# marksho-sfdc/TransmogrifAI

Hardware: AMD Instinct MI355X
Metric: end-to-end AutoML wall-clock + hold-out AuPR, 10M-row binary-class tabular (lower is better)
Workload: dtype fp32; 1 GPU; binary-10m; model=BinaryClassificationModelSelector(default grid), rows=10000000, raw_columns=200, cv_folds=3, global_batch=10000000, max_training_sample=1000000, parallelism=single

## Files before the change

### transmogrifai_amd/ops/csrc/hip/tree_kernels.hip

```cpp
#include <hip/hip_runtime.h>
#include <algorithm>
#include <cstdlib>
#include <stdint.h>
#include <math.h>

#define TM_MAX_S 16
#define TM_WIDE_MAX_S 256
#define TM_WIDE_MAX_BS 16384

namespace {

struct HistItem {
  int32_t node;
  int32_t fg0;
  int32_t nf;
  int32_t excl;
  int64_t begin;
  int64_t count;
};

__device__ __forceinline__ uint32_t ent_row(uint32_t e, int wide) { return wide ? e : (e & 0xFFFFFFu); }
__device__ __forceinline__ uint32_t ent_w(uint32_t e, int wide) { return wide ? 1u : (e >> 24); }

template <int MODE>
// ... 513 lines not shown
      const int f = k / (B * S);
      if (k - f * (B * S) >= wlimit) continue;
      const int64_t acc = lds[f * rowstride + (k - f * (B * S))];
      if (excl) out[k] = acc;
      else if (acc != 0) atomicAdd(reinterpret_cast<unsigned long long*>(out + k), (unsigned long long)acc);
    }
    return;
  }
  const int cwords = FG * B * sc;
  for (int k = threadIdx.x; k < cwords; k += blockDim.x) {
    const int f = k / (B * sc);
    const int rem = k - f * (B * sc);
    int64_t acc = 0;
    for (int r = 0; r < R; ++r) acc += lds[(r * FG + f) * rowstride + rem];
    const int bin = rem / sc, c = rem - bin * sc;
    int64_t* w = out + ((int64_t)f * B + bin) * S + s0 + c;
    if (excl) *w = acc;
    else if (acc != 0) atomicAdd(reinterpret_cast<unsigned long long*>(w), (unsigned long long)acc);
  }
  }
}

__device__ __forceinline__ int64_t live_words(int64_t sz, int64_t dense, int per, int S) {
  return (dense < 0 || sz <= dense) ? sz : dense + (sz - dense) / per * S;
}
__device__ __forceinline__ int live_word(int k, int dense, int per, int S) {
  if (dense < 0 || k < dense) return k;
  const int t = k - dense, f = t / S;
  return dense + f * per + (t - f * S);
}

__global__ void hist_subtract_kernel(int64_t* __restrict__ hist, const int64_t* __restrict__ parent,
                                     const int64_t* __restrict__ parent_off, const int64_t* __restrict__ small_off,
                                     const int64_t* __restrict__ out_off, const int64_t* __restrict__ size, int n,
                                     int64_t dense, int per, int S) {
  const int j = blockIdx.y;
  if (j >= n) return;
  const int sz = (int)live_words(size[j], dense, per, S);
  const int dn = (int)dense;
  const int64_t* p = parent + parent_off[j];
  const int64_t* s = hist + small_off[j];
  int64_t* o = hist + out_off[j];
  for (int k = blockIdx.x * blockDim.x + threadIdx.x; k < sz; k += gridDim.x * blockDim.x) {
    const int w = live_word(k, dn, per, S);
    o[w] = p[w] - s[w];
  }
}

__global__ void zero_segments_kernel(int64_t* __restrict__ hist, const int64_t* __restrict__ off,
                                     const int64_t* __restrict__ size, int n, int64_t dense, int per, int S,
                                     int n_dense, const int* __restrict__ dcnt) {
  const int j = blockIdx.y;
  if (dcnt != nullptr) {
    n = dcnt[0];
    n_dense = dcnt[1];
  }
  if (j >= n) return;
  int64_t* o = hist + off[j];
  const int64_t dj = j < n_dense ? dense : 0;
  const int sz = (int)live_words(size[j], dj, per, S);
  const int dn = (int)dj;
  for (int k = blockIdx.x * blockDim.x + threadIdx.x; k < sz; k += gridDim.x * blockDim.x)
    o[live_word(k, dn, per, S)] = 0;
}

#pragma clang fp contract(off)
__device__ __forceinline__ double impurity_dev(const double* st, int S, int kind, double* cnt) {
  if (kind == 0 || kind == 1) {
    double n = 0;
    for (int s = 0; s < S; ++s) n += st[s];
    *cnt = n;
    if (n <= 0) return 0.0;
    double imp = kind == 0 ? 1.0 : 0.0;
    for (int s = 0; s < S; ++s) {
      const double p = st[s] / n;
      if (kind == 0) imp -= p * p;
      else if (p > 0) imp -= p * log2(p);
    }
    return imp;
  }
  if (kind == 2) {
    const double n = st[0];
    *cnt = n;
    if (n <= 0) return 0.0;
    const double m = st[1] / n;
    return st[2] / n - m * m;
  }
  *cnt = st[1];
  return 0.0;
}

#define TM_FOR_S(s) _Pragma("unroll") for (int s = 0; s < SM; ++s) if (s < S)

template <int SM>
__device__ __forceinline__ double impurity_reg(const double* st, int S, int kind, double* cnt) {
  if (kind == 0 || kind == 1) {
    double n = 0;
    TM_FOR_S(s) n += st[s];
    *cnt = n;
    if (n <= 0) return 0.0;
    double imp = kind == 0 ? 1.0 : 0.0;
    TM_FOR_S(s) {
      const double p = st[s] / n;
      if (kind == 0) imp -= p * p;
      else if (p > 0) imp -= p * log2(p);
    }
    return imp;
  }
  if (kind == 2) {
    const double n = st[0];
    *cnt = n;
    if (n <= 0) return 0.0;
    const double m = st[1] / n;
    return st[2] / n - m * m;
  }
  *cnt = st[1];
  return 0.0;
}

struct Best {
  double gain;
  int f;
  int b;
  int dl;
};
static_assert(sizeof(Best) == 24, "candidate record: three 8-byte words (store_best_sc1 / load_best_sc1)");

__device__ __forceinline__ void store_best_sc1(Best* p, const Best& b) {
  uint64_t* w = reinterpret_cast<uint64_t*>(p);
  __hip_atomic_store(w, (uint64_t)__double_as_longlong(b.gain), __ATOMIC_RELAXED, __HIP_MEMORY_SCOPE_AGENT);
  __hip_atomic_store(w + 1, (uint64_t)(uint32_t)b.f | ((uint64_t)(uint32_t)b.b << 32), __ATOMIC_RELAXED,
                     __HIP_MEMORY_SCOPE_AGENT);
  __hip_atomic_store(w + 2, (uint64_t)(uint32_t)b.dl, __ATOMIC_RELAXED, __HIP_MEMORY_SCOPE_AGENT);
}
__device__ __forceinline__ Best load_best_sc1(const Best* p) {
  const uint64_t* w = reinterpret_cast<const uint64_t*>(p);
  const uint64_t g = __hip_atomic_load(w, __ATOMIC_RELAXED, __HIP_MEMORY_SCOPE_AGENT);
  const uint64_t fb = __hip_atomic_load(w + 1, __ATOMIC_RELAXED, __HIP_MEMORY_SCOPE_AGENT);
  const uint64_t dl = __hip_atomic_load(w + 2, __ATOMIC_RELAXED, __HIP_MEMORY_SCOPE_AGENT);
  return Best{__longlong_as_double((long long)g), (int)(uint32_t)fb, (int)(uint32_t)(fb >> 32), (int)(uint32_t)dl};
}

__device__ __forceinline__ bool better(const Best& a, const Best& b) {
  if (a.gain != b.gain) return a.gain > b.gain;
  if (a.f != b.f) return a.f < b.f;
  if (a.dl != b.dl) return a.dl < b.dl;
  return a.b < b.b;
}

constexpr int FPB = 16;

static inline int cand_stride(int fbmax) { return (fbmax + 15) & ~15; }

static int split_fpb() {
  static const int v = [] {
    const char* e = std::getenv("TMOG_SPLIT_FPB");
    const int x = e ? std::atoi(e) : FPB;
    return (x == 4 || x == 8 || x == 16) ? x : FPB;
  }();
  return v;
}

struct ReduceArgs {
  const int64_t* hist;
  const int64_t* node_hist_off;
  const int32_t* node_feat_off;
  const int32_t* feat_list;
  int B, S, missing_bin;
  const int32_t* node_model;
  const double* qinv;
  int fbmax;
  int cstride;
  const Best* cand;
  int32_t* out_feat;
  int32_t* out_bin;
  float* out_gain;
  uint8_t* out_dl;
  float* out_left;
  float* out_total;
  unsigned long long* cursors;
  uint8_t* rec;
  int64_t rec_bytes;
  int fp_mlo, fp_nml, fp_obase;
};

__device__ __forceinline__ void reduce_node(const ReduceArgs& ra, int j, int lane, bool sc1 = false) {
  const int B = ra.B, S = ra.S, fbmax = ra.fbmax, missing_bin = ra.missing_bin;
  if (ra.cursors && lane < 2) ra.cursors[2 * j + lane] = 0;
  Best b{-INFINITY, 0x7fffffff, 0, 0};
  for (int i = lane; i < fbmax; i += 64) {
    const Best* cp = ra.cand + (int64_t)j * ra.cstride + i;
    const Best c = sc1 ? load_best_sc1(cp) : *cp;
    if (better(c, b)) b = c;
  }
  for (int off = 32; off > 0; off >>= 1) {
    Best o;
    o.gain = __shfl_xor(b.gain, off, 64);
    o.f = __shfl_xor(b.f, off, 64);
    o.b = __shfl_xor(b.b, off, 64);
    o.dl = __shfl_xor(b.dl, off, 64);
    if (better(o, b)) b = o;
  }
  const bool found = b.f != 0x7fffffff && b.gain > -INFINITY;
  const int64_t* h = ra.hist + ra.node_hist_off[j];
  const double* qi = ra.qinv + (int64_t)(ra.node_model ? ra.node_model[j] : 0) * S;
  if (lane == 0) {
    ra.out_feat[j] = found ? ra.feat_list[ra.node_feat_off[j] + b.f] : -1;
    ra.out_bin[j] = found ? b.b : -1;
    ra.out_gain[j] = found ? (float)b.gain : -INFINITY;
    ra.out_dl[j] = (uint8_t)(found ? b.dl : 0);
  }
  for (int s = 0; s < S; ++s) {
    int64_t t = 0, l = 0;
    const int64_t* hf = h + (int64_t)(found ? b.f : 0) * B * S;
    for (int bb = lane; bb < B; bb += 64) {
      t += h[(int64_t)bb * S + s];
      if (found && bb <= b.b) l += hf[(int64_t)bb * S + s];
    }
    if (found && b.dl && lane == 0) l += hf[(int64_t)missing_bin * S + s];
    for (int off = 32; off > 0; off >>= 1) {
      t += __shfl_xor(t, off, 64);
      l += __shfl_xor(l, off, 64);
    }
    if (lane == 0) {
      ra.out_total[(int64_t)j * S + s] = (float)((double)t * qi[s]);
      ra.out_left[(int64_t)j * S + s] = (float)((double)l * qi[s]);
      if (ra.rec) reinterpret_cast<float*>(ra.rec + (int64_t)j * ra.rec_bytes + 24)[s] = (float)((double)l * qi[s]);
    }
  }
  if (ra.rec && lane == 0) {
    uint8_t* r = ra.rec + (int64_t)j * ra.rec_bytes;
    *reinterpret_cast<double*>(r) = found ? b.gain : -INFINITY;
    reinterpret_cast<int32_t*>(r)[2] =
        found ? (b.f < ra.fp_nml ? ra.fp_mlo + b.f : ra.fp_obase + (b.f - ra.fp_nml)) : 0x7fffffff;
    reinterpret_cast<int32_t*>(r)[3] = found ? b.b : -1;
    reinterpret_cast<int32_t*>(r)[4] = found ? b.dl : 0;
    reinterpret_cast<int32_t*>(r)[5] = found ? ra.feat_list[ra.node_feat_off[j] + b.f] : -1;
  }
}

template <int SM>
struct NodeScan {
  int64_t totq[SM];
  double tot[SM], q[SM];
  double tcount, pimp, parent_gain, min_inst, min_gain, mcw, lambda;
  int S, kind;
  bool allow_missing;
  Best best;

  __device__ __forceinline__ void init(const int64_t* totq_in, const double* qi, const float* P, int S_, int kind_,
                                       int missing_bin) {
    S = S_;
    kind = kind_;
    best = Best{-INFINITY, 0x7fffffff, 0, 0};
    min_inst = P[0];
    min_gain = P[1];
    mcw = P[2];
    lambda = P[3];
    allow_missing = P[5] > 0.5f && missing_bin >= 0;
    TM_FOR_S(s) {
      totq[s] = totq_in[s];
      q[s] = qi[s];
      tot[s] = (double)totq[s] * q[s];
    }
    pimp = impurity_reg<SM>(tot, S, kind, &tcount);
    parent_gain = kind == 3 ? tot[0] * tot[0] / (tot[1] + lambda) : 0.0;
  }

  __device__ __forceinline__ void consider(const int64_t* lq, int f, int b, int dl) {
    double left[SM], right[SM];
    TM_FOR_S(s) {
      left[s] = (double)lq[s] * q[s];
      right[s] = (double)(totq[s] - lq[s]) * q[s];
    }
    double gain;
    bool ok = true;
    if (kind == 3) {
      if (left[1] < mcw || right[1] < mcw) return;
      gain = left[0] * left[0] / (left[1] + lambda) + right[0] * right[0] / (right[1] + lambda) - parent_gain;
    } else {
      double lc, rc;
      const double li = impurity_reg<SM>(left, S, kind, &lc);
      const double ri = impurity_reg<SM>(right, S, kind, &rc);
      if (lc < min_inst || rc < min_inst || lc <= 0 || rc <= 0) ok = false;
      gain = pimp - (lc / tcount) * li - (rc / tcount) * ri;
      if (gain < min_gain) ok = false;
    }
    if (ok) {
      Best c{gain, f, b, dl};
      if (better(c, best)) best = c;
    }
  }

  __device__ __forceinline__ void scan_feature(int64_t* v, const int64_t* miss, int nb, int f, int lane) {
    TM_FOR_S(s) v[s] = wave_scan64(v[s]);
    bool any_miss = false;
    TM_FOR_S(s) any_miss |= miss[s] != 0;
    const int n_dl = allow_missing ? (any_miss ? 2 : 1) : 1;
    if (lane < nb - 1 + (allow_missing ? 1 : 0)) {
      for (int dl = 0; dl < n_dl; ++dl) {
        if (lane == nb - 1 && dl) continue;
        int64_t lq[SM];
        TM_FOR_S(s) lq[s] = v[s] + (dl ? miss[s] : 0);
        consider(lq, f, lane, dl);
      }
    }
  }

  __device__ __forceinline__ void wave_best() {
    for (int off = 32; off > 0; off >>= 1) {
      Best o;
      o.gain = __shfl_xor(best.gain, off, 64);
      o.f = __shfl_xor(best.f, off, 64);
      o.b = __shfl_xor(best.b, off, 64);
      o.dl = __shfl_xor(best.dl, off, 64);
      if (better(o, best)) best = o;
    }
  }
};

template <int SM>
__device__ __forceinline__ void node_totals(const int64_t* h, int B, int S, int lane, int64_t* totq) {
  int64_t v[SM];
  TM_FOR_S(s) v[s] = lane < B ? h[lane * S + s] : 0;
  TM_FOR_S(s) totq[s] = readlane64(wave_scan64(v[s]), 63);
}

template <int SM>
__global__ void __launch_bounds__(256) split_scan_kernel(
    const int64_t* __restrict__ hist, const int64_t* __restrict__ node_hist_off, const int32_t* __restrict__ node_nfeat,
    const int32_t* __restrict__ node_feat_off, const int32_t* __restrict__ feat_list,
    const int32_t* __restrict__ feat_nbins, int B, int S, int kind, const float* __restrict__ node_params,
    int missing_bin, const int32_t* __restrict__ node_model, const double* __restrict__ qinv, int fbmax,
    Best* __restrict__ cand, int n_multi, int fpb, unsigned* __restrict__ done, ReduceArgs ra,
    const int* __restrict__ dm) {
  const int cstride = ra.cstride;
  const int j = blockIdx.x / fbmax;
  const int fb = blockIdx.x - j * fbmax;
  if (dm != nullptr && j >= *dm) return;
  const int lane = threadIdx.x & 63, wave = threadIdx.x >> 6;
  if (node_params[(int64_t)j * 8 + 4] > 0.5f) {
    if (done && fb == 0 && wave == 0) reduce_node(ra, j, lane);
    return;
  }
  const int nf = node_nfeat[j];
  const int f_lim = n_multi >= 0 ? min(n_multi, nf) : nf;
  const int fb_multi = n_multi >= 0 ? (n_multi + fpb - 1) / fpb : fbmax;
  const bool one_blk = fb >= fb_multi;
  __shared__ Best s_best[4];
  NodeScan<SM> ns;
  ns.best = Best{-INFINITY, 0x7fffffff, 0, 0};
  if (node_params[(int64_t)j * 8 + 7] > 0.5f &&
      (one_blk ? (n_multi + (fb - fb_multi) * 256 < nf) : (fb * fpb < f_lim))) {
    const int64_t* h = hist + node_hist_off[j];
    const int32_t* fl = feat_list + node_feat_off[j];
    int64_t totq[SM];
    node_totals<SM>(h, B, S, lane, totq);
    ns.init(totq, qinv + (int64_t)(node_model ? node_model[j] : 0) * S, node_params + (int64_t)j * 8, S, kind,
            missing_bin);
    const int f_end = one_blk ? 0 : min(f_lim, (fb + 1) * fpb);
    if (one_blk) {
      const int f = n_multi + (fb - fb_multi) * 256 + (int)threadIdx.x;
      if (f < nf && ns.allow_missing && feat_nbins[fl[f]] == 1) {
        const int64_t* hf = h + (int64_t)f * B * S;
        int64_t lq[SM];
        TM_FOR_S(s) lq[s] = hf[s];
        ns.consider(lq, f, 0, 0);
      }
    }
    for (int f = fb * fpb + wave; f < f_end; f += 4) {
      const int nb = feat_nbins[fl[f]];
      const int64_t* hf = h + (int64_t)f * B * S;
      if (nb == 1) {
        if (ns.allow_missing && lane == 0) {
          int64_t lq[SM];
          TM_FOR_S(s) lq[s] = hf[s];
          ns.consider(lq, f, 0, 0);
        }
        continue;
      }
      int64_t v[SM], miss[SM];
      const int bl = lane < nb ? lane : 0;
      const int mbin = missing_bin >= 0 ? missing_bin : 0;
      TM_FOR_S(s) {
        v[s] = hf[bl * S + s];
        miss[s] = hf[mbin * S + s];
      }
      TM_FOR_S(s) {
        v[s] = lane < nb ? v[s] : 0;
        miss[s] = ns.allow_missing ? miss[s] : 0;
      }
      ns.scan_feature(v, miss, nb, f, lane);
    }
  }
  ns.wave_best();
  if (lane == 0) s_best[wave] = ns.best;
  __syncthreads();
  if (done == nullptr) {
    if (threadIdx.x == 0) {
      Best b = s_best[0];
      for (int w = 1; w < 4; ++w)
        if (better(s_best[w], b)) b = s_best[w];
      cand[(int64_t)j * cstride + fb] = b;
    }
    return;
  }
  if (wave == 0) {
    unsigned last = 0;
    if (lane == 0) {
      Best b = s_best[0];
      for (int w = 1; w < 4; ++w)
        if (better(s_best[w], b)) b = s_best[w];
      store_best_sc1(cand + (int64_t)j * cstride + fb, b);
      asm volatile("s_waitcnt vmcnt(0)" ::: "memory");
      last = __hip_atomic_fetch_add(done + j, 1u, __ATOMIC_RELAXED, __HIP_MEMORY_SCOPE_AGENT) ==
             (unsigned)(fbmax - 1);
    }
    last = __shfl(last, 0, 64);
    if (last) {
      reduce_node(ra, j, lane, true);
      if (lane == 0) __hip_atomic_store(done + j, 0u, __ATOMIC_RELAXED, __HIP_MEMORY_SCOPE_AGENT);
    }
  }
}

template <int SM>
__global__ void __launch_bounds__(256) pair_scan_kernel(
    int64_t* __restrict__ hist, const int64_t* __restrict__ parent, const int64_t* __restrict__ parent_off,
    const int32_t* __restrict__ small_j, const int32_t* __restrict__ big_j, int n_pairs,
    const int64_t* __restrict__ node_hist_off, const int32_t* __restrict__ node_nfeat,
    const int32_t* __restrict__ node_feat_off, const int32_t* __restrict__ feat_list,
    const int32_t* __restrict__ feat_nbins, int B, int S, int kind, const float* __restrict__ node_params,
    int missing_bin, const int32_t* __restrict__ node_model, const double* __restrict__ qinv, int fbmax,
    Best* __restrict__ cand, int n_multi, int fpb, int cstride, const int* __restrict__ dnp) {
  const int q = blockIdx.x / fbmax;
  const int fb = blockIdx.x - q * fbmax;
  if (dnp != nullptr) n_pairs = *dnp;
  if (q >= n_pairs) return;
  const int lane = threadIdx.x & 63, wave = threadIdx.x >> 6;
  const int js = small_j[q], jb = big_j[q];
  const int nf = node_nfeat[js];
  const int f_lim = n_multi >= 0 ? min(n_multi, nf) : nf;
  const int fb_multi = n_multi >= 0 ? (n_multi + fpb - 1) / fpb : fbmax;
  const bool one_blk = fb >= fb_multi;
  const int64_t* P = parent + parent_off[q];
  const int64_t* Hs = hist + node_hist_off[js];
  int64_t* Hb = hist + node_hist_off[jb];
  const int32_t* fl = feat_list + node_feat_off[js];
  const bool scan_s = node_params[(int64_t)js * 8 + 7] > 0.5f;
  const bool scan_b = node_params[(int64_t)jb * 8 + 7] > 0.5f;
  __shared__ Best s_best[2][4];
  NodeScan<SM> ns, nb_;
  {
    int64_t ts[SM], tp[SM], tb[SM];
    node_totals<SM>(Hs, B, S, lane, ts);
    node_totals<SM>(P, B, S, lane, tp);
    TM_FOR_S(s) tb[s] = tp[s] - ts[s];
    ns.init(ts, qinv + (int64_t)(node_model ? node_model[js] : 0) * S, node_params + (int64_t)js * 8, S, kind,
            missing_bin);
    nb_.init(tb, qinv + (int64_t)(node_model ? node_model[jb] : 0) * S, node_params + (int64_t)jb * 8, S, kind,
             missing_bin);
  }
  if (one_blk) {
    const int f = n_multi + (fb - fb_multi) * 256 + (int)threadIdx.x;
    if (f < nf) {
      const int64_t o = (int64_t)f * B * S;
      int64_t ls[SM], lb[SM];
      TM_FOR_S(s) {
        ls[s] = Hs[o + s];
        lb[s] = P[o + s] - ls[s];
        Hb[o + s] = lb[s];
      }
      if (feat_nbins[fl[f]] == 1) {
        if (scan_s && ns.allow_missing) ns.consider(ls, f, 0, 0);
        if (scan_b && nb_.allow_missing) nb_.consider(lb, f, 0, 0);
      }
    }
  } else {
    const int f_end = min(f_lim, (fb + 1) * fpb);
    for (int f = fb * fpb + wave; f < f_end; f += 4) {
      const int nbins = feat_nbins[fl[f]];
      const int64_t o = (int64_t)f * B * S;
      int64_t vs[SM], vb[SM], ms[SM], mb[SM], pa[SM], pp[SM];
      const int bl = lane < B ? lane : 0;
      TM_FOR_S(s) {
        pa[s] = Hs[o + bl * S + s];
        pp[s] = P[o + bl * S + s];
      }
      TM_FOR_S(s) {
        const int64_t a = lane < B ? pa[s] : 0;
        const int64_t c = lane < B ? pp[s] - pa[s] : 0;
        if (lane < B) Hb[o + lane * S + s] = c;
        ms[s] = missing_bin >= 0 ? readlane64(a, missing_bin) : 0;
        mb[s] = missing_bin >= 0 ? readlane64(c, missing_bin) : 0;
        vs[s] = lane < nbins ? a : 0;
        vb[s] = lane < nbins ? c : 0;
      }
      if (nbins == 1) {
        if (lane == 0) {
          if (scan_s && ns.allow_missing) ns.consider(vs, f, 0, 0);
          if (scan_b && nb_.allow_missing) nb_.consider(vb, f, 0, 0);
        }
        continue;
      }
      if (scan_s) {
        if (!ns.allow_missing)
          TM_FOR_S(s) ms[s] = 0;
        ns.scan_feature(vs, ms, nbins, f, lane);
      }
      if (scan_b) {
        if (!nb_.allow_missing)
          TM_FOR_S(s) mb[s] = 0;
        nb_.scan_feature(vb, mb, nbins, f, lane);
      }
    }
  }
  ns.wave_best();
  nb_.wave_best();
  if (lane == 0) {
    s_best[0][wave] = ns.best;
    s_best[1][wave] = nb_.best;
  }
  __syncthreads();
  if (threadIdx.x < 2) {
    Best b = s_best[threadIdx.x][0];
    for (int w = 1; w < 4; ++w)
      if (better(s_best[threadIdx.x][w], b)) b = s_best[threadIdx.x][w];
    cand[(int64_t)(threadIdx.x ? jb : js) * cstride + fb] = b;
  }
}

__global__ void __launch_bounds__(256) split_scan_wide_kernel(
    const int64_t* __restrict__ hist, const int64_t* __restrict__ node_hist_off, const int32_t* __restrict__ node_nfeat,
    const int32_t* __restrict__ node_feat_off, const int32_t* __restrict__ feat_list,
    const int32_t* __restrict__ feat_nbins, int B, int S, int kind, const float* __restrict__ node_params,
    int missing_bin, const int32_t* __restrict__ node_model, const double* __restrict__ qinv, int fbmax,
    Best* __restrict__ cand, int n_multi, int cstride) {
  extern __shared__ __attribute__((aligned(16))) int64_t wl[];
  int64_t* H = wl;
  int64_t* totq = H + (int64_t)B * S;
  int64_t* miss = totq + S;
  double* q = reinterpret_cast<double*>(miss + S);
  __shared__ Best s_best[4];
  const int j = blockIdx.x / fbmax;
  const int f = blockIdx.x - j * fbmax;
  const int nf = node_nfeat[j];
  Best best{-INFINITY, 0x7fffffff, 0, 0};
  const bool live = f < nf && node_params[(int64_t)j * 8 + 7] > 0.5f;
  const int64_t* h = hist + node_hist_off[j];
  const int32_t* fl = feat_list + node_feat_off[j];
  const float* P = node_params + (int64_t)j * 8;
  const double* qi = qinv + (int64_t)(node_model ? node_model[j] : 0) * S;
  const double min_inst = P[0], min_gain = P[1], mcw = P[2], lambda = P[3];
  const bool allow_missing = P[5] > 0.5f && missing_bin >= 0;
  const int nb = live ? feat_nbins[fl[f]] : 0;
  const bool one = live && n_multi >= 0 && f >= n_multi;
  const int64_t* hf = h + (int64_t)f * B * S;
  if (live) {
    for (int i = threadIdx.x; i < B * S; i += blockDim.x) H[i] = (one && i >= S) ? 0 : hf[i];
    for (int s = threadIdx.x; s < S; s += blockDim.x) {
      int64_t t = 0;
      for (int bb = 0; bb < B; ++bb) t += h[(int64_t)bb * S + s];
      totq[s] = t;
      miss[s] = allow_missing ? hf[(int64_t)missing_bin * S + s] : 0;
      q[s] = qi[s];
    }
  }
  __syncthreads();
  if (live)
    for (int s = threadIdx.x; s < S; s += blockDim.x)
      for (int bb = 1; bb < B; ++bb) H[(int64_t)bb * S + s] += H[(int64_t)(bb - 1) * S + s];
  __syncthreads();
  if (live) {
    double tcount = 0, pimp = 0, parent_gain = 0;
    if (kind == 0 || kind == 1) {
      for (int s = 0; s < S; ++s) tcount += (double)totq[s] * q[s];
      if (tcount > 0) {
        pimp = kind == 0 ? 1.0 : 0.0;
        for (int s = 0; s < S; ++s) {
          const double p = ((double)totq[s] * q[s]) / tcount;
          if (kind == 0) pimp -= p * p;
          else if (p > 0) pimp -= p * log2(p);
        }
      }
    } else {
      double tot[4] = {0, 0, 0, 0};
      for (int s = 0; s < S && s < 4; ++s) tot[s] = (double)totq[s] * q[s];
      pimp = impurity_dev(tot, S, kind, &tcount);
      parent_gain = kind == 3 ? tot[0] * tot[0] / (tot[1] + lambda) : 0.0;
    }
    const int nd = allow_missing ? 2 : 1;
    const int nbc = one ? 1 : nb - 1 + (allow_missing ? 1 : 0);
    for (int c = threadIdx.x; c < nbc * nd; c += blockDim.x) {
      const int dl = c / nbc, b = one ? 0 : c - dl * nbc;
      if (one && (dl || !allow_missing)) continue;
      if (!one && b == nb - 1 && dl) continue;
      const int64_t* lp = H + (int64_t)b * S;
      double gain;
      bool ok = true;
      if (kind == 0 || kind == 1) {
        double lc = 0, rc = 0;
        for (int s = 0; s < S; ++s) {
          const int64_t lq = lp[s] + (dl ? miss[s] : 0);
          lc += (double)lq * q[s];
          rc += (double)(totq[s] - lq) * q[s];
        }
        double li = 0, ri = 0;
        if (lc > 0) {
          li = kind == 0 ? 1.0 : 0.0;
          for (int s = 0; s < S; ++s) {
            const double p = ((double)(lp[s] + (dl ? miss[s] : 0)) * q[s]) / lc;
            if (kind == 0) li -= p * p;
            else if (p > 0) li -= p * log2(p);
          }
        }
        if (rc > 0) {
          ri = kind == 0 ? 1.0 : 0.0;
          for (int s = 0; s < S; ++s) {
            const double p = ((double)(totq[s] - lp[s] - (dl ? miss[s] : 0)) * q[s]) / rc;
            if (kind == 0) ri -= p * p;
            else if (p > 0) ri -= p * log2(p);
          }
        }
        if (lc < min_inst || rc < min_inst || lc <= 0 || rc <= 0) ok = false;
        gain = pimp - (lc / tcount) * li - (rc / tcount) * ri;
        if (gain < min_gain) ok = false;
      } else {
        double left[4] = {0, 0, 0, 0}, right[4] = {0, 0, 0, 0};
        for (int s = 0; s < S && s < 4; ++s) {
          const int64_t lq = lp[s] + (dl ? miss[s] : 0);
          left[s] = (double)lq * q[s];
          right[s] = (double)(totq[s] - lq) * q[s];
        }
        if (kind == 3) {
          if (left[1] < mcw || right[1] < mcw) ok = false;
          gain = left[0] * left[0] / (left[1] + lambda) + right[0] * right[0] / (right[1] + lambda) - parent_gain;
        } else {
          double lc, rc;
          const double li = impurity_dev(left, S, kind, &lc);
          const double ri = impurity_dev(right, S, kind, &rc);
          if (lc < min_inst || rc < min_inst || lc <= 0 || rc <= 0) ok = false;
          gain = pimp - (lc / tcount) * li - (rc / tcount) * ri;
          if (gain < min_gain) ok = false;
        }
      }
      if (ok) {
        const Best cb{gain, f, b, dl};
        if (better(cb, best)) best = cb;
      }
    }
  }
  const int lane = threadIdx.x & 63, wave = threadIdx.x >> 6;
  for (int off = 32; off > 0; off >>= 1) {
    Best o;
    o.gain = __shfl_xor(best.gain, off, 64);
    o.f = __shfl_xor(best.f, off, 64);
    o.b = __shfl_xor(best.b, off, 64);
    o.dl = __shfl_xor(best.dl, off, 64);
    if (better(o, best)) best = o;
  }
  if (lane == 0) s_best[wave] = best;
  __syncthreads();
  if (threadIdx.x == 0) {
    Best bb = s_best[0];
    for (int w = 1; w < 4; ++w)
      if (better(s_best[w], bb)) bb = s_best[w];
    cand[(int64_t)j * cstride + f] = bb;
// ... 344 lines not shown
      active = false;
#pragma unroll
      for (int u = 0; u < 4; ++u) {
        if (nd[u].z >= 0) {
          const uint8_t b = xr[nd[u].x];
          const bool gl = (missing_bin >= 0 && b == missing_bin) ? (default_left[k[u]] != 0) : ((int)b <= nd[u].y);
          k[u] = gl ? nd[u].z : nd[u].w;
          nd[u] = nodes[k[u]];
          active = true;
        }
      }
    }
#pragma unroll
    for (int u = 0; u < 4; ++u) {
      const float w = tree_weight[t + u];
      for (int c = 0; c < K && c < 8; ++c) acc[c] += w * leaf_value[k[u] * K + c];
    }
  }
  for (; t < t_end; ++t) {
    int64_t k = tree_off[t];
    int4 nd = nodes[k];
    while (nd.z >= 0) {
      const uint8_t b = xr[nd.x];
      const bool gl = (missing_bin >= 0 && b == missing_bin) ? (default_left[k] != 0) : ((int)b <= nd.y);
      k = gl ? nd.z : nd.w;
      nd = nodes[k];
    }
    const float w = tree_weight[t];
    for (int c = 0; c < K && c < 8; ++c) acc[c] += w * leaf_value[k * K + c];
  }
  float* o = out + i * K;
  for (int c = 0; c < K && c < 8; ++c) o[c] = acc[c];
}

}

extern "C" {

int tmog_hip_debug_flags(int flags) {
  return (int)hipMemcpyToSymbol(HIP_SYMBOL(g_hist_debug), &flags, sizeof(int));
}

int tmog_hip_hist_build(const uint8_t* Xb, int F, const uint32_t* rows, const void* items, int n_items,
                        const int32_t* node_feat_off, const int32_t* feat_list, const int32_t* node_model,
                        const int64_t* node_hist_off, int64_t* hist, int B, int mode, int S, const float* y,
                        const float* t1, const float* t2, int64_t stride, const float* qscale, int skip_bin,
                        const int64_t* csr_ptr, const uint16_t* csr_col, int Sc, int n_wide, int need_general,
                        hipStream_t stream, const int32_t* gh_words, const int* dcount, int wide_rows,
                        const uint8_t* Xh, int Fh) {
  if (n_items == 0) return 0;
  if (Xh == nullptr) {
    Xh = Xb;
    Fh = F;
  }
  if (dcount != nullptr && n_wide != 0) return -2;
  const int2* gh = reinterpret_cast<const int2*>(gh_words);
  if (gh && mode != 2) return -2;
  if (Sc <= 0 || Sc > S) Sc = S;
  size_t lds = (size_t)(((64 * (B * Sc + 1)) + 3) & ~3) * sizeof(int) + 4 * 64 * sizeof(int4) +
               TM_MAX_S * sizeof(int);
  if (mode == 2 && S == 2) {
    const size_t wl = (size_t)((2 * (64 * (B + 1) + 17) + 3) & ~3) * sizeof(int) + 4 * 64 * sizeof(int4) +
                      4 * sizeof(int);
    if (wl > lds) lds = wl;
  }
  if (lds > 160 * 1024) return -2;
  if (skip_bin >= B || (mode == 2 && skip_bin >= 0 && (S != 2 || Sc != S))) return -2;
  if (mode == 0 && S > TM_WIDE_MAX_S) return -2;
  if ((csr_ptr != nullptr) != (csr_col != nullptr) || (csr_ptr && (mode != 2 || skip_bin <= 0))) return -2;
  const HistItem* it = (const HistItem*)items;
  if (n_wide < 0 || n_wide > n_items || (n_wide > 0 && (mode != 2 || S != 2))) return -2;
  static const bool split_wide = [] { const char* e = std::getenv("TMOG_HIST_WIDE_SPLIT"); return e && e[0] == '1'; }();
  if (!split_wide) n_wide = 0;
  if (n_wide > 0) {
    static const int occ = [] { const char* e = std::getenv("TMOG_HIST_WIDE_OCC"); return e ? std::atoi(e) : 6; }();
    if (occ >= 7)
      hipLaunchKernelGGL(hist_wide_kernel<7>, dim3(n_wide), dim3(256), lds, stream, Xb, F, rows, it, node_feat_off,
                         feat_list, node_model, node_hist_off, hist, B, t1, t2, stride, qscale, skip_bin, gh, wide_rows, Xh, Fh);
    else
      hipLaunchKernelGGL(hist_wide_kernel<6>, dim3(n_wide), dim3(256), lds, stream, Xb, F, rows, it, node_feat_off,
                         feat_list, node_model, node_hist_off, hist, B, t1, t2, stride, qscale, skip_bin, gh, wide_rows, Xh, Fh);
    it += n_wide;
    n_items -= n_wide;
    if (n_items == 0) return (int)hipGetLastError();
  }
  dim3 grid(n_items), block(256);
  if (mode == 0)
    hipLaunchKernelGGL(hist_build_kernel<0>, grid, block, lds, stream, Xb, F, rows, it, node_feat_off, feat_list,
                       node_model, node_hist_off, hist, B, S, y, t1, t2, stride, qscale, -1, nullptr, nullptr, Sc,
                       nullptr, dcount, wide_rows, Xh, Fh);
  else if (mode == 1)
    hipLaunchKernelGGL(hist_build_kernel<1>, grid, block, lds, stream, Xb, F, rows, it, node_feat_off, feat_list,
                       node_model, node_hist_off, hist, B, S, y, t1, t2, stride, qscale, -1, nullptr, nullptr, Sc,
                       nullptr, dcount, wide_rows, Xh, Fh);
  else if (need_general)
    hipLaunchKernelGGL(hist_build_kernel<2>, grid, block, lds, stream, Xb, F, rows, it, node_feat_off, feat_list,
                       node_model, node_hist_off, hist, B, S, y, t1, t2, stride, qscale, skip_bin, csr_ptr,
                       csr_col, Sc, gh, dcount, wide_rows, Xh, Fh);
  else
    hipLaunchKernelGGL((hist_build_kernel<2, false>), grid, block, lds, stream, Xb, F, rows, it, node_feat_off,
                       feat_list, node_model, node_hist_off, hist, B, S, y, t1, t2, stride, qscale, skip_bin, csr_ptr,
                       csr_col, Sc, gh, dcount, wide_rows, Xh, Fh);
  return (int)hipGetLastError();
}

static int64_t host_live_words(int64_t sz, int64_t dense, int per, int S) {
  return (dense < 0 || sz <= dense) ? sz : dense + (sz - dense) / per * S;
}

int tmog_hip_hist_subtract(int64_t* hist, const int64_t* parent, const int64_t* parent_off, const int64_t* small_off,
                           const int64_t* out_off, const int64_t* size, int n, int64_t max_size, int64_t dense,
                           int per, int S, hipStream_t stream) {
  if (n == 0) return 0;
  if (max_size >= (int64_t)1 << 31) return -2;
  int gx = (int)min((host_live_words(max_size, dense, per, S) + 255) / 256, (int64_t)1024);
  if (gx < 1) gx = 1;
  hipLaunchKernelGGL(hist_subtract_kernel, dim3(gx, n), dim3(256), 0, stream, hist, parent, parent_off, small_off,
                     out_off, size, n, dense, per, S);
  return (int)hipGetLastError();
}

int tmog_hip_split_find(const int64_t* hist, int n_nodes, const int64_t* node_hist_off, const int32_t* node_nfeat,
                        const int32_t* node_feat_off, const int32_t* feat_list, const int32_t* feat_nbins, int B,
                        int S, int kind, const float* node_params, int missing_bin, const int32_t* node_model,
                        const double* qinv, int max_nfeat, void* cand_ws, int32_t* out_feat, int32_t* out_bin,
                        float* out_gain, uint8_t* out_dl, float* out_left, float* out_total, int64_t* cursors,
                        int n_multi, void* rec, int64_t rec_bytes, int fp_mlo, int fp_nml, int fp_obase,
                        hipStream_t stream, unsigned* done, const int* dm) {
  if (n_nodes == 0) return 0;
  if (dm != nullptr && (done == nullptr || S > TM_MAX_S || B > 64)) return -2;
  if (n_multi > max_nfeat) n_multi = -1;
  Best* cand = (Best*)cand_ws;
  const bool wide = S > TM_MAX_S || B > 64;
  int fbmax;
  auto make_ra = [&](int fbm) {
    return ReduceArgs{hist, node_hist_off, node_feat_off, feat_list, B, S, missing_bin, node_model, qinv, fbm,
                      cand_stride(fbm), cand,
                      out_feat, out_bin, out_gain, out_dl, out_left, out_total, (unsigned long long*)cursors,
                      (uint8_t*)rec, rec_bytes, fp_mlo, fp_nml, fp_obase};
  };
  ReduceArgs ra{};
  if (wide) {
    if (S > TM_WIDE_MAX_S || B * S > TM_WIDE_MAX_BS) return -2;
    fbmax = max_nfeat;
    const size_t lds = ((size_t)B * S + 3 * (size_t)S) * 8;
    hipLaunchKernelGGL(split_scan_wide_kernel, dim3(n_nodes * fbmax), dim3(256), lds, stream, hist, node_hist_off,
                       node_nfeat, node_feat_off, feat_list, feat_nbins, B, S, kind, node_params, missing_bin,
                       node_model, qinv, fbmax, cand, n_multi, cand_stride(fbmax));
  } else {
  const int fpb = split_fpb();
  fbmax = n_multi >= 0 ? (n_multi + fpb - 1) / fpb + (max_nfeat - n_multi + 255) / 256
                       : (max_nfeat + fpb - 1) / fpb;
  ra = make_ra(fbmax);
#define TM_SPLIT(SMV)                                                                                          \
  hipLaunchKernelGGL(split_scan_kernel<SMV>, dim3(n_nodes * fbmax), dim3(256), 0, stream, hist, node_hist_off,  \
                     node_nfeat, node_feat_off, feat_list, feat_nbins, B, S, kind, node_params, missing_bin,    \
                     node_model, qinv, fbmax, cand, n_multi, fpb, done, ra, dm)
  if (S <= 2) TM_SPLIT(2);
  else if (S == 3) TM_SPLIT(3);
  else if (S <= 4) TM_SPLIT(4);
  else TM_SPLIT(TM_MAX_S);
#undef TM_SPLIT
  }
  if (wide) ra = make_ra(fbmax);
  if (wide || done == nullptr)
    hipLaunchKernelGGL(split_reduce_kernel, dim3(n_nodes), dim3(64), 0, stream, ra);
  return (int)hipGetLastError();
}

int tmog_hip_pair_scan(int64_t* hist, const int64_t* parent, const int64_t* parent_off, const int32_t* small_j,
                       const int32_t* big_j, int n_pairs, const int64_t* node_hist_off, const int32_t* node_nfeat,
                       const int32_t* node_feat_off, const int32_t* feat_list, const int32_t* feat_nbins, int B, int S,
                       int kind, const float* node_params, int missing_bin, const int32_t* node_model,
                       const double* qinv, int max_nfeat, void* cand_ws, int n_multi, hipStream_t stream,
                       const int* dnp) {
  if (n_pairs == 0) return 0;
  if (S > TM_MAX_S || B > 64) return -2;
  if (n_multi > max_nfeat) n_multi = -1;
  const int fpb = split_fpb();
  const int fbmax = n_multi >= 0 ? (n_multi + fpb - 1) / fpb + (max_nfeat - n_multi + 255) / 256
                                 : (max_nfeat + fpb - 1) / fpb;
#define TM_PAIR(SMV)                                                                                           \
  hipLaunchKernelGGL(pair_scan_kernel<SMV>, dim3(n_pairs * fbmax), dim3(256), 0, stream, hist, parent, parent_off, \
                     small_j, big_j, n_pairs, node_hist_off, node_nfeat, node_feat_off, feat_list, feat_nbins, B, S, \
                     kind, node_params, missing_bin, node_model, qinv, fbmax, (Best*)cand_ws, n_multi, fpb,    \
                     cand_stride(fbmax), dnp)
  if (S <= 2) TM_PAIR(2);
  else if (S == 3) TM_PAIR(3);
  else if (S <= 4) TM_PAIR(4);
  else TM_PAIR(TM_MAX_S);
#undef TM_PAIR
  return (int)hipGetLastError();
}

int tmog_hip_fp_merge(const void* recv, int R, int m, int64_t rec_bytes, int S, int32_t* out_feat, int32_t* out_bin,
                      float* out_gain, uint8_t* out_dl, float* out_left, hipStream_t stream) {
  if (m == 0) return 0;
  hipLaunchKernelGGL(fp_merge_kernel, dim3((m + 255) / 256), dim3(256), 0, stream, (const uint8_t*)recv, R, m,
                     rec_bytes, S, out_feat, out_bin, out_gain, out_dl, out_left, (int64_t)m, (const int*)nullptr);
  return (int)hipGetLastError();
}

int tmog_hip_fp_merge_dev(const void* recv, int R, int m_stride, int64_t rec_bytes, int S, int32_t* out_feat,
                          int32_t* out_bin, float* out_gain, uint8_t* out_dl, float* out_left, const int* dm,
                          hipStream_t stream) {
  if (m_stride == 0) return 0;
  hipLaunchKernelGGL(fp_merge_kernel, dim3((m_stride + 255) / 256), dim3(256), 0, stream, (const uint8_t*)recv, R,
                     m_stride, rec_bytes, S, out_feat, out_bin, out_gain, out_dl, out_left, (int64_t)m_stride, dm);
  return (int)hipGetLastError();
}

int tmog_hip_zero_segments(int64_t* hist, const int64_t* off, const int64_t* size, int n, int64_t max_size,
                           int64_t dense, int per, int S, hipStream_t stream, int n_dense, const int* dn) {
  if (n == 0) return 0;
  if (max_size >= (int64_t)1 << 31) return -2;
  const int64_t lw = std::max(host_live_words(max_size, dense, per, S), host_live_words(max_size, 0, per, S));
  int gx = (int)min((lw + 255) / 256, (int64_t)1024);
  if (gx < 1) gx = 1;
  hipLaunchKernelGGL(zero_segments_kernel, dim3(gx, n), dim3(256), 0, stream, hist, off, size, n, dense, per, S,
                     n_dense, dn);
  return (int)hipGetLastError();
}

int tmog_hip_tree_prime() {
  hipFuncAttributes at;
  return (int)hipFuncGetAttributes(&at, reinterpret_cast<const void*>(&zero_segments_kernel));
}

size_t tmog_hip_split_cand_bytes(int n_nodes, int max_nfeat, int B, int S) {
  const bool wide = S > TM_MAX_S || B > 64;
  const int fpb = split_fpb();
  return (size_t)n_nodes * cand_stride(wide ? max_nfeat : (max_nfeat + fpb - 1) / fpb + 1) * sizeof(Best);
}

int tmog_hip_hist_stat_chunk(int B, int S) {
  int sc = S;
  while (sc > 1 && (size_t)(((64 * (B * sc + 1)) + 3) & ~3) * sizeof(int) + 4 * 64 * sizeof(int4) +
                       TM_MAX_S * sizeof(int) > 160 * 1024)
    --sc;
  return sc;
}

int tmog_hip_partition_fused(const uint8_t* Xb, int F, const uint32_t* rows_in, uint32_t* rows_out, const void* items,
                             int n_items, const int64_t* node_begin, const int64_t* node_count, const int32_t* split_feat,
                             const int32_t* split_bin, const uint8_t* dl, const float* node_params,
                             const float* split_gain, int missing_bin, int64_t* cursors, const uint8_t* XbT,
                             int64_t N, hipStream_t stream, const int32_t* gh_in, int32_t* gh_out, const int* dcount,
                             int wide_rows) {
  if (n_items == 0) return 0;
  if ((gh_in != nullptr) != (gh_out != nullptr)) return -2;
  hipLaunchKernelGGL(partition_fused_kernel, dim3(n_items), dim3(256), 0, stream, Xb, F, rows_in, rows_out,
                     (const PartItem*)items, node_begin, node_count, split_feat, split_bin, dl, node_params,
                     split_gain, missing_bin, (unsigned long long*)cursors, XbT, N,
                     reinterpret_cast<const int2*>(gh_in), reinterpret_cast<int2*>(gh_out), dcount, wide_rows);
  return (int)hipGetLastError();
}

int tmog_hip_leaf_collect(const uint32_t* rows, const void* items, int n_items, uint32_t* out_rows,
                          int32_t* out_gid, hipStream_t stream, const uint32_t* rows_alt, const int* dcount) {
  if (n_items == 0) return 0;
  hipLaunchKernelGGL(leaf_collect_kernel, dim3(n_items), dim3(256), 0, stream, rows, rows_alt, (const LeafItem*)items,
                     out_rows, out_gid, dcount);
  return (int)hipGetLastError();
}

int tmog_hip_forest_predict_multi(const uint8_t* Xb, int F, int n_models, const int64_t* model_row_off,
                                  const int32_t* row_list, int64_t max_rows, const int64_t* model_tree_off,
                                  const int64_t* tree_off, const float* tree_weight, const int32_t* nodes,
                                  const uint8_t* default_left, int missing_bin, const float* leaf_value, int K,
                                  const uint32_t* node_mask, const int32_t* var_off, const int32_t* var_depth,
                                  const int64_t* var_out_off, float* out, hipStream_t stream) {
  if (n_models == 0 || max_rows == 0) return 0;
  if (K != 1 && K != 2 && K != 4 && K != 8) return -2;
  const size_t lds = (((size_t)PM_ROWS * F + 15) & ~(size_t)15) + sizeof(float) * PM_VK * PM_ROWS * PM_TPR;
  if (lds > 160 * 1024) return -3;
  dim3 g2((unsigned)((max_rows + PM_ROWS - 1) / PM_ROWS), n_models);
#define TM_PM(KV)                                                                                               \
  hipLaunchKernelGGL(forest_predict_multi_kernel<KV>, g2, dim3(PM_ROWS * PM_TPR), lds, stream, Xb, F,           \
                     model_row_off, row_list, model_tree_off, tree_off, tree_weight, (const int4*)nodes,         \
                     default_left, missing_bin, leaf_value, K, node_mask, var_off, var_depth, var_out_off,      \
                     out)
  if (K == 1) TM_PM(1);
  else if (K == 2) TM_PM(2);
  else if (K == 4) TM_PM(4);
  else TM_PM(8);
#undef TM_PM
  return (int)hipGetLastError();
}

int tmog_hip_forest_predict(const uint8_t* Xb, int F, int n_models, const int64_t* model_row_off,
                            const int32_t* row_list, int64_t max_rows, const int64_t* model_tree_off,
                            const int64_t* tree_off, const float* tree_weight, const int32_t* nodes,
                            const uint8_t* default_left, int missing_bin, const float* leaf_value, int K, float* out,
                            hipStream_t stream) {
  if (n_models == 0 || max_rows == 0) return 0;
  if (K > 8) return -2;
  if ((size_t)PRED_ROWS * F <= 64 * 1024) {
    dim3 g2((unsigned)((max_rows + PRED_ROWS - 1) / PRED_ROWS), n_models);
    const size_t lds = (((size_t)PRED_ROWS * F + 15) & ~(size_t)15) + sizeof(float) * 8 * PRED_ROWS * PRED_TPR;
    hipLaunchKernelGGL(forest_predict_lds_kernel, g2, dim3(PRED_ROWS * PRED_TPR), lds, stream, Xb, F,
                       model_row_off, row_list, model_tree_off, tree_off, tree_weight, (const int4*)nodes,
                       default_left, missing_bin, leaf_value, K, out);
    return (int)hipGetLastError();
  }
  dim3 grid((unsigned)((max_rows + 255) / 256), n_models);
  hipLaunchKernelGGL(forest_predict_kernel, grid, dim3(256), 0, stream, Xb, F, model_row_off, row_list,
                     model_tree_off, tree_off, tree_weight, (const int4*)nodes, default_left, missing_bin, leaf_value,
                     K, out);
  return (int)hipGetLastError();
}

}
```

Baseline: 1.678 s per end-to-end AutoML train.

## Add Newton-specialized split scan kernels with software-prefetched histogram rows

Adds a NEWTON template specialization of the split and pair scan kernels. It is used for gradient-boosting (kind 3, S=2) by default and can be disabled with an env var. The specialization compiles out impurity code, pins the wave index and per-pair indices into scalar registers, and double-buffers the next feature's histogram row and bin count while the current one is scanned, using sched_barrier to hold the ordering. The aim is to hide global load latency and cut per-iteration branching in the split search, at the cost of extra registers and more template instantiations.

Result: faster. 1.616 s per end-to-end AutoML train, median of 6 (-3.7%).

```diff
diff --git a/transmogrifai_amd/ops/csrc/hip/tree_kernels.hip b/transmogrifai_amd/ops/csrc/hip/tree_kernels.hip
--- a/transmogrifai_amd/ops/csrc/hip/tree_kernels.hip
+++ b/transmogrifai_amd/ops/csrc/hip/tree_kernels.hip
@@ -689,6 +689,12 @@
 
 static inline int cand_stride(int fbmax) { return (fbmax + 15) & ~15; }
 
+static bool scan_newton(int kind, int S) {
+  if (kind != 3 || S != 2) return false;
+  const char* e = std::getenv("TMOG_SCAN_GENERIC");
+  return !(e && e[0] == '1');
+}
+
 static int split_fpb() {
   static const int v = [] {
     const char* e = std::getenv("TMOG_SPLIT_FPB");
@@ -776,7 +782,7 @@
   }
 }
 
-template <int SM>
+template <int SM, bool NEWTON = false>
 struct NodeScan {
   int64_t totq[SM];
   double tot[SM], q[SM];
@@ -788,7 +794,7 @@
   __device__ __forceinline__ void init(const int64_t* totq_in, const double* qi, const float* P, int S_, int kind_,
                                        int missing_bin) {
     S = S_;
-    kind = kind_;
+    kind = NEWTON ? 3 : kind_;
     best = Best{-INFINITY, 0x7fffffff, 0, 0};
     min_inst = P[0];
     min_gain = P[1];
@@ -800,8 +806,12 @@
       q[s] = qi[s];
       tot[s] = (double)totq[s] * q[s];
     }
-    pimp = impurity_reg<SM>(tot, S, kind, &tcount);
-    parent_gain = kind == 3 ? tot[0] * tot[0] / (tot[1] + lambda) : 0.0;
+    if constexpr (NEWTON) {
+      parent_gain = tot[0] * tot[0] / (tot[1] + lambda);
+    } else {
+      pimp = impurity_reg<SM>(tot, S, kind, &tcount);
+      parent_gain = kind == 3 ? tot[0] * tot[0] / (tot[1] + lambda) : 0.0;
+    }
   }
 
   __device__ __forceinline__ void consider(const int64_t* lq, int f, int b, int dl) {
@@ -812,10 +822,10 @@
     }
     double gain;
     bool ok = true;
-    if (kind == 3) {
+    if (NEWTON || kind == 3) {
       if (left[1] < mcw || right[1] < mcw) return;
       gain = left[0] * left[0] / (left[1] + lambda) + right[0] * right[0] / (right[1] + lambda) - parent_gain;
-    } else {
+    } else if constexpr (!NEWTON) {
       double lc, rc;
       const double li = impurity_reg<SM>(left, S, kind, &lc);
       const double ri = impurity_reg<SM>(right, S, kind, &rc);
@@ -864,6 +874,27 @@
 }
 
 template <int SM>
+__device__ __forceinline__ void load_row(const int64_t* __restrict__ h, int f, int B, int S, int lane, int64_t* v) {
+  const int64_t o = (int64_t)f * B * S + (lane < B ? lane : 0) * S;
+  TM_FOR_S(s) v[s] = h[o + s];
+}
+
+template <class T>
+__device__ __forceinline__ void pin_scalar(T& v) {
+  asm volatile("" : "+s"(v));
+}
+template <class... T>
+__device__ __forceinline__ void batch_end(T&... v) {
+  __builtin_amdgcn_sched_barrier(0);
+  (pin_scalar(v), ...);
+}
+
+template <int SM>
+__device__ __forceinline__ void row_totals(const int64_t* row, int B, int S, int lane, int64_t* totq) {
+  TM_FOR_S(s) totq[s] = readlane64(wave_scan64(lane < B ? row[s] : 0), 63);
+}
+
+template <int SM, bool NEWTON>
 __global__ void __launch_bounds__(256) split_scan_kernel(
     const int64_t* __restrict__ hist, const int64_t* __restrict__ node_hist_off, const int32_t* __restrict__ node_nfeat,
     const int32_t* __restrict__ node_feat_off, const int32_t* __restrict__ feat_list,
@@ -872,10 +903,12 @@
     Best* __restrict__ cand, int n_multi, int fpb, unsigned* __restrict__ done, ReduceArgs ra,
     const int* __restrict__ dm) {
   const int cstride = ra.cstride;
+  if constexpr (NEWTON) S = SM;
   const int j = blockIdx.x / fbmax;
   const int fb = blockIdx.x - j * fbmax;
   if (dm != nullptr && j >= *dm) return;
-  const int lane = threadIdx.x & 63, wave = threadIdx.x >> 6;
+  const int lane = threadIdx.x & 63;
+  const int wave = NEWTON ? __builtin_amdgcn_readfirstlane(threadIdx.x >> 6) : (int)(threadIdx.x >> 6);
   if (node_params[(int64_t)j * 8 + 4] > 0.5f) {
     if (done && fb == 0 && wave == 0) reduce_node(ra, j, lane);
     return;
@@ -885,17 +918,34 @@
   const int fb_multi = n_multi >= 0 ? (n_multi + fpb - 1) / fpb : fbmax;
   const bool one_blk = fb >= fb_multi;
   __shared__ Best s_best[4];
-  NodeScan<SM> ns;
+  NodeScan<SM, NEWTON> ns;
   ns.best = Best{-INFINITY, 0x7fffffff, 0, 0};
   if (node_params[(int64_t)j * 8 + 7] > 0.5f &&
       (one_blk ? (n_multi + (fb - fb_multi) * 256 < nf) : (fb * fpb < f_lim))) {
     const int64_t* h = hist + node_hist_off[j];
     const int32_t* fl = feat_list + node_feat_off[j];
+    const int f_end = one_blk ? 0 : min(f_lim, (fb + 1) * fpb);
+    const int mbin = missing_bin >= 0 ? missing_bin : 0;
+    [[maybe_unused]] int64_t nv[SM], nm[SM];
+    [[maybe_unused]] int nb_next = 0;
+    [[maybe_unused]] auto issue = [&](int f) {
+      load_row<SM>(h, f, B, S, lane, nv);
+      const int64_t* hf = h + (int64_t)f * B * S;
+      TM_FOR_S(s) nm[s] = hf[mbin * S + s];
+      nb_next = feat_nbins[fl[f]];
+    };
     int64_t totq[SM];
-    node_totals<SM>(h, B, S, lane, totq);
+    if constexpr (NEWTON) {
+      int64_t r0[SM];
+      load_row<SM>(h, 0, B, S, lane, r0);
+      if (fb * fpb + wave < f_end) issue(fb * fpb + wave);
+      __builtin_amdgcn_sched_barrier(0);
+      row_totals<SM>(r0, B, S, lane, totq);
+    } else {
+      node_totals<SM>(h, B, S, lane, totq);
+    }
     ns.init(totq, qinv + (int64_t)(node_model ? node_model[j] : 0) * S, node_params + (int64_t)j * 8, S, kind,
             missing_bin);
-    const int f_end = one_blk ? 0 : min(f_lim, (fb + 1) * fpb);
     if (one_blk) {
       const int f = n_multi + (fb - fb_multi) * 256 + (int)threadIdx.x;
       if (f < nf && ns.allow_missing && feat_nbins[fl[f]] == 1) {
@@ -905,29 +955,50 @@
         ns.consider(lq, f, 0, 0);
       }
     }
-    for (int f = fb * fpb + wave; f < f_end; f += 4) {
-      const int nb = feat_nbins[fl[f]];
-      const int64_t* hf = h + (int64_t)f * B * S;
-      if (nb == 1) {
-        if (ns.allow_missing && lane == 0) {
-          int64_t lq[SM];
-          TM_FOR_S(s) lq[s] = hf[s];
-          ns.consider(lq, f, 0, 0);
+    if constexpr (NEWTON) {
+      for (int f = fb * fpb + wave; f < f_end; f += 4) {
+        int64_t v[SM], miss[SM];
+        const int nb = nb_next;
+        TM_FOR_S(s) {
+          v[s] = nv[s];
+          miss[s] = nm[s];
         }
-        continue;
-      }
-      int64_t v[SM], miss[SM];
-      const int bl = lane < nb ? lane : 0;
-      const int mbin = missing_bin >= 0 ? missing_bin : 0;
-      TM_FOR_S(s) {
-        v[s] = hf[bl * S + s];
-        miss[s] = hf[mbin * S + s];
-      }
-      TM_FOR_S(s) {
-        v[s] = lane < nb ? v[s] : 0;
-        miss[s] = ns.allow_missing ? miss[s] : 0;
-      }
-      ns.scan_feature(v, miss, nb, f, lane);
+        if (f + 4 < f_end) issue(f + 4);
+        __builtin_amdgcn_sched_barrier(0);
+        if (nb == 1) {
+          if (ns.allow_missing && lane == 0) ns.consider(v, f, 0, 0);
+          continue;
+        }
+        TM_FOR_S(s) {
+          v[s] = lane < nb ? v[s] : 0;
+          miss[s] = ns.allow_missing ? miss[s] : 0;
+        }
+        ns.scan_feature(v, miss, nb, f, lane);
+      }
+    } else {
+      for (int f = fb * fpb + wave; f < f_end; f += 4) {
+        const int nb = feat_nbins[fl[f]];
+        const int64_t* hf = h + (int64_t)f * B * S;
+        if (nb == 1) {
+          if (ns.allow_missing && lane == 0) {
+            int64_t lq[SM];
+            TM_FOR_S(s) lq[s] = hf[s];
+            ns.consider(lq, f, 0, 0);
+          }
+          continue;
+        }
+        int64_t v[SM], miss[SM];
+        const int bl = lane < nb ? lane : 0;
+        TM_FOR_S(s) {
+          v[s] = hf[bl * S + s];
+          miss[s] = hf[mbin * S + s];
+        }
+        TM_FOR_S(s) {
+          v[s] = lane < nb ? v[s] : 0;
+          miss[s] = ns.allow_missing ? miss[s] : 0;
+        }
+        ns.scan_feature(v, miss, nb, f, lane);
+      }
     }
   }
   ns.wave_best();
@@ -961,7 +1032,7 @@
   }
 }
 
-template <int SM>
+template <int SM, bool NEWTON>
 __global__ void __launch_bounds__(256) pair_scan_kernel(
     int64_t* __restrict__ hist, const int64_t* __restrict__ parent, const int64_t* __restrict__ parent_off,
     const int32_t* __restrict__ small_j, const int32_t* __restrict__ big_j, int n_pairs,
@@ -970,34 +1041,88 @@
     const int32_t* __restrict__ feat_nbins, int B, int S, int kind, const float* __restrict__ node_params,
     int missing_bin, const int32_t* __restrict__ node_model, const double* __restrict__ qinv, int fbmax,
     Best* __restrict__ cand, int n_multi, int fpb, int cstride, const int* __restrict__ dnp) {
+  if constexpr (NEWTON) S = SM;
   const int q = blockIdx.x / fbmax;
   const int fb = blockIdx.x - q * fbmax;
   if (dnp != nullptr) n_pairs = *dnp;
   if (q >= n_pairs) return;
-  const int lane = threadIdx.x & 63, wave = threadIdx.x >> 6;
-  const int js = small_j[q], jb = big_j[q];
-  const int nf = node_nfeat[js];
+  const int lane = threadIdx.x & 63;
+  const int wave = NEWTON ? __builtin_amdgcn_readfirstlane(threadIdx.x >> 6) : (int)(threadIdx.x >> 6);
+  int js = small_j[q], jb = big_j[q];
+  int64_t poff = parent_off[q];
+  if constexpr (NEWTON) batch_end(js, jb, poff);
+  int nf = node_nfeat[js];
+  int64_t hs_off = node_hist_off[js], hb_off = node_hist_off[jb];
+  int fl_off = node_feat_off[js];
+  float may_s = node_params[(int64_t)js * 8 + 7], may_b = node_params[(int64_t)jb * 8 + 7];
+  if constexpr (NEWTON) batch_end(nf, hs_off, hb_off, fl_off, may_s, may_b);
+  const int64_t* P = parent + poff;
+  const int64_t* Hs = hist + hs_off;
+  int64_t* Hb = hist + hb_off;
+  const int32_t* fl = feat_list + fl_off;
+  const bool scan_s = may_s > 0.5f, scan_b = may_b > 0.5f;
   const int f_lim = n_multi >= 0 ? min(n_multi, nf) : nf;
   const int fb_multi = n_multi >= 0 ? (n_multi + fpb - 1) / fpb : fbmax;
   const bool one_blk = fb >= fb_multi;
-  const int64_t* P = parent + parent_off[q];
-  const int64_t* Hs = hist + node_hist_off[js];
-  int64_t* Hb = hist + node_hist_off[jb];
-  const int32_t* fl = feat_list + node_feat_off[js];
-  const bool scan_s = node_params[(int64_t)js * 8 + 7] > 0.5f;
-  const bool scan_b = node_params[(int64_t)jb * 8 + 7] > 0.5f;
+  const int f_end = one_blk ? 0 : min(f_lim, (fb + 1) * fpb);
+  [[maybe_unused]] int64_t na[SM], np_[SM];
+  [[maybe_unused]] int nb_next = 0;
+  [[maybe_unused]] auto issue = [&](int f) {
+    load_row<SM>(Hs, f, B, S, lane, na);
+    load_row<SM>(P, f, B, S, lane, np_);
+    nb_next = feat_nbins[fl[f]];
+  };
   __shared__ Best s_best[2][4];
-  NodeScan<SM> ns, nb_;
+  NodeScan<SM, NEWTON> ns, nb_;
   {
     int64_t ts[SM], tp[SM], tb[SM];
-    node_totals<SM>(Hs, B, S, lane, ts);
-    node_totals<SM>(P, B, S, lane, tp);
+    if constexpr (NEWTON) {
+      int64_t rs[SM], rp[SM];
+      load_row<SM>(Hs, 0, B, S, lane, rs);
+      load_row<SM>(P, 0, B, S, lane, rp);
+      if (fb * fpb + wave < f_end) issue(fb * fpb + wave);
+      __builtin_amdgcn_sched_barrier(0);
+      row_totals<SM>(rs, B, S, lane, ts);
+      row_totals<SM>(rp, B, S, lane, tp);
+    } else {
+      node_totals<SM>(Hs, B, S, lane, ts);
+      node_totals<SM>(P, B, S, lane, tp);
+    }
     TM_FOR_S(s) tb[s] = tp[s] - ts[s];
-    ns.init(ts, qinv + (int64_t)(node_model ? node_model[js] : 0) * S, node_params + (int64_t)js * 8, S, kind,
-            missing_bin);
-    nb_.init(tb, qinv + (int64_t)(node_model ? node_model[jb] : 0) * S, node_params + (int64_t)jb * 8, S, kind,
-             missing_bin);
-  }
+    const int model_s = node_model ? node_model[js] : 0, model_b = node_model ? node_model[jb] : 0;
+    ns.init(ts, qinv + (int64_t)model_s * S, node_params + (int64_t)js * 8, S, kind, missing_bin);
+    nb_.init(tb, qinv + (int64_t)model_b * S, node_params + (int64_t)jb * 8, S, kind, missing_bin);
+  }
+  auto scan_pair = [&](int f, int nbins, const int64_t* pa, const int64_t* pp) {
+    const int64_t o = (int64_t)f * B * S;
+    int64_t vs[SM], vb[SM], ms[SM], mb[SM];
+    TM_FOR_S(s) {
+      const int64_t a = lane < B ? pa[s] : 0;
+      const int64_t c = lane < B ? pp[s] - pa[s] : 0;
+      if (lane < B) Hb[o + lane * S + s] = c;
+      ms[s] = missing_bin >= 0 ? readlane64(a, missing_bin) : 0;
+      mb[s] = missing_bin >= 0 ? readlane64(c, missing_bin) : 0;
+      vs[s] = lane < nbins ? a : 0;
+      vb[s] = lane < nbins ? c : 0;
+    }
+    if (nbins == 1) {
+      if (lane == 0) {
+        if (scan_s && ns.allow_missing) ns.consider(vs, f, 0, 0);
+        if (scan_b && nb_.allow_missing) nb_.consider(vb, f, 0, 0);
+      }
+      return;
+    }
+    if (scan_s) {
+      if (!ns.allow_missing)
+        TM_FOR_S(s) ms[s] = 0;
+      ns.scan_feature(vs, ms, nbins, f, lane);
+    }
+    if (scan_b) {
+      if (!nb_.allow_missing)
+        TM_FOR_S(s) mb[s] = 0;
+      nb_.scan_feature(vb, mb, nbins, f, lane);
+    }
+  };
   if (one_blk) {
     const int f = n_multi + (fb - fb_multi) * 256 + (int)threadIdx.x;
     if (f < nf) {
@@ -1013,43 +1138,25 @@
         if (scan_b && nb_.allow_missing) nb_.consider(lb, f, 0, 0);
       }
     }
+  } else if constexpr (NEWTON) {
+    for (int f = fb * fpb + wave; f < f_end; f += 4) {
+      int64_t pa[SM], pp[SM];
+      const int nbins = nb_next;
+      TM_FOR_S(s) {
+        pa[s] = na[s];
+        pp[s] = np_[s];
+      }
+      if (f + 4 < f_end) issue(f + 4);
+      __builtin_amdgcn_sched_barrier(0);
+      scan_pair(f, nbins, pa, pp);
+    }
   } else {
-    const int f_end = min(f_lim, (fb + 1) * fpb);
     for (int f = fb * fpb + wave; f < f_end; f += 4) {
       const int nbins = feat_nbins[fl[f]];
-      const int64_t o = (int64_t)f * B * S;
-      int64_t vs[SM], vb[SM], ms[SM], mb[SM], pa[SM], pp[SM];
-      const int bl = lane < B ? lane : 0;
-      TM_FOR_S(s) {
-        pa[s] = Hs[o + bl * S + s];
-        pp[s] = P[o + bl * S + s];
-      }
-      TM_FOR_S(s) {
-        const int64_t a = lane < B ? pa[s] : 0;
-        const int64_t c = lane < B ? pp[s] - pa[s] : 0;
-        if (lane < B) Hb[o + lane * S + s] = c;
-        ms[s] = missing_bin >= 0 ? readlane64(a, missing_bin) : 0;
-        mb[s] = missing_bin >= 0 ? readlane64(c, missing_bin) : 0;
-        vs[s] = lane < nbins ? a : 0;
-        vb[s] = lane < nbins ? c : 0;
-      }
-      if (nbins == 1) {
-        if (lane == 0) {
-          if (scan_s && ns.allow_missing) ns.consider(vs, f, 0, 0);
-          if (scan_b && nb_.allow_missing) nb_.consider(vb, f, 0, 0);
-        }
-        continue;
-      }
-      if (scan_s) {
-        if (!ns.allow_missing)
-          TM_FOR_S(s) ms[s] = 0;
-        ns.scan_feature(vs, ms, nbins, f, lane);
-      }
-      if (scan_b) {
-        if (!nb_.allow_missing)
-          TM_FOR_S(s) mb[s] = 0;
-        nb_.scan_feature(vb, mb, nbins, f, lane);
-      }
+      int64_t pa[SM], pp[SM];
+      load_row<SM>(Hs, f, B, S, lane, pa);
+      load_row<SM>(P, f, B, S, lane, pp);
+      scan_pair(f, nbins, pa, pp);
     }
   }
   ns.wave_best();
@@ -1700,14 +1807,15 @@
   fbmax = n_multi >= 0 ? (n_multi + fpb - 1) / fpb + (max_nfeat - n_multi + 255) / 256
                        : (max_nfeat + fpb - 1) / fpb;
   ra = make_ra(fbmax);
-#define TM_SPLIT(SMV)                                                                                          \
-  hipLaunchKernelGGL(split_scan_kernel<SMV>, dim3(n_nodes * fbmax), dim3(256), 0, stream, hist, node_hist_off,  \
+#define TM_SPLIT(...)                                                                                          \
+  hipLaunchKernelGGL((split_scan_kernel<__VA_ARGS__>), dim3(n_nodes * fbmax), dim3(256), 0, stream, hist, node_hist_off,  \
                      node_nfeat, node_feat_off, feat_list, feat_nbins, B, S, kind, node_params, missing_bin,    \
                      node_model, qinv, fbmax, cand, n_multi, fpb, done, ra, dm)
-  if (S <= 2) TM_SPLIT(2);
-  else if (S == 3) TM_SPLIT(3);
-  else if (S <= 4) TM_SPLIT(4);
-  else TM_SPLIT(TM_MAX_S);
+  if (scan_newton(kind, S)) TM_SPLIT(2, true);
+  else if (S <= 2) TM_SPLIT(2, false);
+  else if (S == 3) TM_SPLIT(3, false);
+  else if (S <= 4) TM_SPLIT(4, false);
+  else TM_SPLIT(TM_MAX_S, false);
 #undef TM_SPLIT
   }
   if (wide) ra = make_ra(fbmax);
@@ -1728,15 +1836,16 @@
   const int fpb = split_fpb();
   const int fbmax = n_multi >= 0 ? (n_multi + fpb - 1) / fpb + (max_nfeat - n_multi + 255) / 256
                                  : (max_nfeat + fpb - 1) / fpb;
-#define TM_PAIR(SMV)                                                                                           \
-  hipLaunchKernelGGL(pair_scan_kernel<SMV>, dim3(n_pairs * fbmax), dim3(256), 0, stream, hist, parent, parent_off, \
+#define TM_PAIR(...)                                                                                           \
+  hipLaunchKernelGGL((pair_scan_kernel<__VA_ARGS__>), dim3(n_pairs * fbmax), dim3(256), 0, stream, hist, parent, parent_off, \
                      small_j, big_j, n_pairs, node_hist_off, node_nfeat, node_feat_off, feat_list, feat_nbins, B, S, \
                      kind, node_params, missing_bin, node_model, qinv, fbmax, (Best*)cand_ws, n_multi, fpb,    \
                      cand_stride(fbmax), dnp)
-  if (S <= 2) TM_PAIR(2);
-  else if (S == 3) TM_PAIR(3);
-  else if (S <= 4) TM_PAIR(4);
-  else TM_PAIR(TM_MAX_S);
+  if (scan_newton(kind, S)) TM_PAIR(2, true);
+  else if (S <= 2) TM_PAIR(2, false);
+  else if (S == 3) TM_PAIR(3, false);
+  else if (S <= 4) TM_PAIR(4, false);
+  else TM_PAIR(TM_MAX_S, false);
 #undef TM_PAIR
   return (int)hipGetLastError();
 }
```
